# pastas/metran

Measured on AMD Instinct MI355X. Metric: Kalman filter+smoother steps/sec (batched DFMs), higher is better.
Workload: dtype f64

## Files before the change

### metran_amd/csrc/mk_kernels.hip

```cpp
#include <cstdlib>
#include <cstring>

#include "mk_prims.h"

namespace mk {

template <int n, int G, bool SYM>
struct RecordIO;
#ifndef MK_WIDE_FILTER_WAVES
#define MK_WIDE_FILTER_WAVES 2
#endif
#ifndef MK_WIDE_FILTER_LOOP
#define MK_WIDE_FILTER_LOOP 1
#endif
#ifndef MK_FILTER_LDS_STORES
#define MK_FILTER_LDS_STORES 1
#endif

template <int N, int K, int G, int OUT, bool BOOK, bool SYM>
__global__ void __launch_bounds__(256) __attribute__((amdgpu_waves_per_eu(G == 64 && N + K <= 40 ? MK_WIDE_FILTER_WAVES : 1))) filter_kernel(FilterArgs a)
{
    static_assert(!SYM || OUT == 1 || OUT == 3, "packed-symmetric layout applies to record outputs");
    constexpr int n = N + K;
    static_assert(n <= G, "state dimension must fit the lane group");
    constexpr bool TAPE = (OUT == 4);
    static_assert(!TAPE || (G == 64 && MK_WIDE_FILTER_LOOP && N * K > 32), "the tape leaves the one-model-per-wavefront loop filter");
    using Gp = Group<G>;
    constexpr int GPB = 256 / G;
    constexpr bool HOIST = (N * K <= 32);
    constexpr int NV = record_payload(n);
    const int lane = threadIdx.x % G;
    long inst = (long)blockIdx.x * GPB + threadIdx.x / G;
    if (inst > a.B - 1) inst = a.B - 1;
    const long rec = inst % a.R;
    const int r = lane < n ? lane : n - 1;
    const bool lead = lane == 0;
    const long T = a.T;

    const double phi_r = a.phi[inst * n + r];
    const double q_r = a.q[inst * n + r];
    constexpr bool WIDE = (G == 64);
    double pp[WIDE ? 1 : n], qd[WIDE ? 1 : n];
    constexpr int NP = n + (n & 1);
    __shared__ __attribute__((aligned(16))) double lds_phi[WIDE ? (256 / G) * 3 * NP : 1];
    double *phim = lds_phi + (WIDE ? (threadIdx.x / G) * 3 * NP : 0);
    double *dvec = phim + (WIDE ? NP : 0);
    double *dvec2 = dvec;
    if constexpr (WIDE) {
        phim[r] = phi_r;
        wave_lds_sync();
    } else {
        sfor<0, n>(MK_LAMBDA(c) {
            pp[decltype(c)::value] = phi_r * Gp::template bcast<decltype(c)::value>(phi_r);
            qd[decltype(c)::value] = (decltype(c)::value == r) ? q_r : 0.0;
        });
    }
    const int jr = lane < N ? lane : N - 1;
    double gam[K];
#pragma unroll
    for (int k = 0; k < K; ++k) gam[k] = a.loadings[(rec * N + jr) * K + k];
    const double rvar = a.obsvar ? a.obsvar[rec * N + jr] : 0.0;
    constexpr bool GTAB = WIDE && !HOIST;
    __shared__ __attribute__((aligned(16))) double lds_gam[GTAB ? (256 / G) * N * K : 1];
    double *gtab = lds_gam + (GTAB ? (threadIdx.x / G) * N * K : 0);
    if constexpr (GTAB) {
        if (lane < N) {
#pragma unroll
            for (int k = 0; k < K; ++k) gtab[lane * K + k] = gam[k];
        }
        wave_lds_sync();
    }
    double Gh[HOIST ? N : 1][K];
    if constexpr (HOIST) {
        sfor<0, N>(MK_LAMBDA(j) {
            sfor<0, K>(MK_LAMBDA(k) {
                Gh[decltype(j)::value][decltype(k)::value] = Gp::template bcast<decltype(j)::value>(gam[decltype(k)::value]);
            });
        });
    }

    double x = a.x0 ? a.x0[inst * n + r] : 0.0;
    double P[n];
#pragma unroll
    for (int c = 0; c < n; ++c) P[c] = a.P0 ? a.P0[(inst * n + r) * n + c] : (c == r ? 1.0 : 0.0);

    constexpr bool XREP = WIDE && MK_WIDE_FILTER_LOOP;
    double xk[XREP ? K : 1], phik[XREP ? K : 1];
    if constexpr (XREP) {
        sfor<0, K>(MK_LAMBDA(k) {
            xk[decltype(k)::value] = Gp::template bcast<N + decltype(k)::value>(x);
            phik[decltype(k)::value] = Gp::template bcast<N + decltype(k)::value>(phi_r);
        });
    }

    constexpr bool RECF = (OUT == 1 || OUT == 3);
    MomentPtr oP = moment_ptr<n>(a.Xp, a.Pp, inst * a.bs, a.ts, OUT == 1 ? a.rs : 0, r);
    MomentPtr oF = moment_ptr<n>(a.F, a.Pf, inst * a.bs, a.ts, RECF ? a.rs : 0, r);
    constexpr int RS = SYM ? record_stride_sym_c(n) : record_stride_c(n), NVO = SYM ? record_payload_sym(n) : NV;
    constexpr int PADN = RS - NVO;
    const int pslot = lane < PADN ? lane : PADN - 1;
    double *padF = RECF ? a.F + inst * a.bs * RS + NVO + pslot : nullptr;
    double *padP = OUT == 1 ? a.Xp + inst * a.bs * RS + NVO + pslot : nullptr;
    constexpr bool LDSOUT = MK_FILTER_LDS_STORES && RECF && G == 16;
    using RIO = RecordIO<n, G, SYM>;
    __shared__ __attribute__((aligned(16))) double lds_rec[LDSOUT ? 4 * 2 * RIO::LDS_PER_WAVE : 1];
    double *imgP = lds_rec + (LDSOUT ? (threadIdx.x / 64) * 2 * RIO::LDS_PER_WAVE : 0);
    double *imgF = imgP + (LDSOUT ? RIO::LDS_PER_WAVE : 0);
    const int lane64 = threadIdx.x & 63, gw = lane64 / G;
    typename RIO::Map rmap;
    double *recP = a.Xp, *recF = a.F;
    const long rstep = a.ts * RS;
    if constexpr (LDSOUT) {
        rmap = RIO::make_map(lane64, (long)blockIdx.x * GPB + (threadIdx.x / 64) * RIO::GW, a.B, a.bs);
        RIO::clear_tail(imgP, lane64);
        RIO::clear_tail(imgF, lane64);
        RIO::put_pad(imgP, gw, 0.0, 0.0);
    }
    double pad0 = 0.0, pad1 = 0.0;
    [[maybe_unused]] constexpr int XS = tape_xs_c(N, K);
    [[maybe_unused]] double *trec = TAPE ? a.F + inst * a.bs * a.rs : nullptr;
    [[maybe_unused]] const long tstep = a.ts * a.rs;

    constexpr int TS = 16;
    const int lrow = lane < TS ? lane : TS - 1;
    constexpr bool OV2 = (N % 2 == 0);
    constexpr int ONC = OV2 ? N / 2 : N;
    using ochunk_t = typename std::conditional<OV2, v2d, double>::type;
    __shared__ __attribute__((aligned(16))) double lds_obs[(256 / G) * TS * N];
    double *otile = lds_obs + (threadIdx.x / G) * TS * N;
    const double *obase = a.obs + rec * a.obs_bs * N;
    const long ostep = a.obs_ts * N;
    ochunk_t oreg[WIDE ? 1 : ONC];
    long otr = 0;
    auto obs_issue = [&](long t0) __attribute__((always_inline)) {
        long tr = t0 + lrow;
        if (tr > T - 1) tr = T - 1;
        if constexpr (WIDE) {
            otr = tr;
        } else {
            const ochunk_t *src = reinterpret_cast<const ochunk_t *>(obase + tr * ostep);
#pragma unroll
            for (int i = 0; i < ONC; ++i) oreg[i] = src[i];
        }
    };
    auto obs_park = [&]() __attribute__((always_inline)) {
        ochunk_t *dst = reinterpret_cast<ochunk_t *>(otile + lrow * N);
        wave_lds_sync();
        if constexpr (WIDE) {
            const ochunk_t *src = reinterpret_cast<const ochunk_t *>(obase + otr * ostep);
#pragma unroll
            for (int i = 0; i < ONC; ++i) dst[i] = src[i];
        } else {
#pragma unroll
            for (int i = 0; i < ONC; ++i) dst[i] = oreg[i];
        }
        wave_lds_sync();
    };
    obs_issue(0);
    double ynext = 0.0;

    double sum_sig = 0.0, sum_det = 0.0;
    double run_mant = 1.0;
    long run_exp = 0;
    long nobs = 0, sc = 0;
    double fmin_seen = 1.0;

    for (long t0 = 0; t0 < T; t0 += TS) {
    obs_park();
    obs_issue(t0 + TS);
    ynext = otile[jr];
    const long tend = t0 + TS < T ? t0 + TS : T;
    for (long t = t0; t < tend; ++t) {
        const double y = ynext;
        {
            const int s1 = (int)(t - t0) + 1;
            ynext = otile[(s1 < TS ? s1 : TS - 1) * N + jr];
        }
        const unsigned long long ball = __ballot(lane < N && isfinite(y));
        const auto vm = Gp::group_bits(ball);

        x = phi_r * x;
        if constexpr (XREP) {
#pragma unroll
            for (int k = 0; k < K; ++k) xk[k] = phik[k] * xk[k];
        }
        if constexpr (WIDE) {
            int rv = r;
            double qv = q_r;
            asm volatile("" : "+v"(rv), "+v"(qv));
            double phc[n];
            load_row<n>(phim, phc);
#pragma unroll
            for (int c = 0; c < n; ++c) P[c] = fma(P[c] * phi_r, phc[c], c == rv ? qv : 0.0);
        } else {
#pragma unroll
            for (int c = 0; c < n; ++c) P[c] = fma(P[c], pp[c], qd[c]);
        }
        if constexpr (LDSOUT && OUT == 1) {
            RIO::put(imgP, gw, r, x, P);
        } else if constexpr (OUT == 1) {
            *oP.vec = x;
            if constexpr (SYM) store_cols_sym<n>(oP.mat - r, P, r);
            else store_cols<n>(oP.mat, P);
            *padP = 0.0;
            oP.advance_nn(1);
            padP += a.ts * RS;
        } else if constexpr (OUT == 2) {
            if (oP.vec) *oP.vec = x;
            if (oP.mat) store_cols<n>(oP.mat, P);
            oP.advance(1);
        }

        double sigma = 0.0, fmant = 1.0;
        int fexp = 0;
        auto update = MK_LAMBDA(jc) {
            constexpr int j = decltype(jc)::value;
            double vl = y - x;
            sfor<0, K>(MK_LAMBDA(k) {
                constexpr int kk = decltype(k)::value;
                Gp::template fmac<N + kk, true>(vl, x, gam[kk]);
            });
            const double v = Gp::template bcast<j>(vl);
            double dr = P[j];
            sfor<0, K>(MK_LAMBDA(k) {
                constexpr int kk = decltype(k)::value;
                double g;
                if constexpr (HOIST) g = Gh[j][kk];
                else if constexpr (GTAB) g = gtab[j * K + kk];
                else g = Gp::template bcast<j>(gam[kk]);
                dr = fma(P[N + kk], g, dr);
            });
            double fl = rvar + dr;
            if constexpr (G == 16) dpp_pin(dr);
            sfor<0, K>(MK_LAMBDA(k) {
                constexpr int kk = decltype(k)::value;
                Gp::template fmac<N + kk, false>(fl, dr, gam[kk]);
            });
            const double f = Gp::template bcast<j>(fl);
            const double rf = rcp_nr(f);
            const double kr = dr * rf;
            if constexpr (WIDE) {
                dvec[r] = dr;
                wave_lds_sync();
                double dc[n];
                load_row<n>(dvec, dc);
#pragma unroll
                for (int c = 0; c < n; ++c) P[c] = fma(-dc[c], kr, P[c]);
            } else {
                Gp::template axpy_col<0, n, true, n>(P, dr, kr);
            }
            x = fma(kr, v, x);
            sigma = fma(v * v, rf, sigma);
            fmant *= f;
            if constexpr ((j & 3) == 3 || j == N - 1) {
                fexp += __builtin_amdgcn_frexp_exp(fmant);
                fmant = __builtin_amdgcn_frexp_mant(fmant);
            }
            fmin_seen = min_f64(fmin_seen, f);
        };
        if constexpr (WIDE && MK_WIDE_FILTER_LOOP) {
            unsigned long long m = (unsigned long long)vm;
            int nupd = 0;
            while (m) {
                const int j = __builtin_amdgcn_readfirstlane((int)__builtin_ctzll(m));
                m &= m - 1;
                double vl = y - x, vl2 = 0.0;
                sfor<0, K>(MK_LAMBDA(k) {
                    constexpr int kk = decltype(k)::value;
                    if constexpr (kk % 2 == 0) vl = fma(-gam[kk], xk[kk], vl);
                    else vl2 = fma(-gam[kk], xk[kk], vl2);
                });
                vl += vl2;
                const double v = readlane_f64(vl, j);
                double dr = 0.0;
                switch (j) {
#define MK_CASE_P(c) \
    case c:          \
        if constexpr (c < N) dr = P[c]; \
        break;
                    MK_CASE_P(0) MK_CASE_P(1) MK_CASE_P(2) MK_CASE_P(3) MK_CASE_P(4) MK_CASE_P(5) MK_CASE_P(6) MK_CASE_P(7)
                    MK_CASE_P(8) MK_CASE_P(9) MK_CASE_P(10) MK_CASE_P(11) MK_CASE_P(12) MK_CASE_P(13) MK_CASE_P(14) MK_CASE_P(15)
                    MK_CASE_P(16) MK_CASE_P(17) MK_CASE_P(18) MK_CASE_P(19) MK_CASE_P(20) MK_CASE_P(21) MK_CASE_P(22) MK_CASE_P(23)
                    MK_CASE_P(24) MK_CASE_P(25) MK_CASE_P(26) MK_CASE_P(27) MK_CASE_P(28) MK_CASE_P(29) MK_CASE_P(30) MK_CASE_P(31)
                    MK_CASE_P(32) MK_CASE_P(33) MK_CASE_P(34) MK_CASE_P(35) MK_CASE_P(36) MK_CASE_P(37) MK_CASE_P(38) MK_CASE_P(39)
                    MK_CASE_P(40) MK_CASE_P(41) MK_CASE_P(42) MK_CASE_P(43) MK_CASE_P(44) MK_CASE_P(45) MK_CASE_P(46) MK_CASE_P(47)
                    MK_CASE_P(48) MK_CASE_P(49) MK_CASE_P(50) MK_CASE_P(51) MK_CASE_P(52) MK_CASE_P(53) MK_CASE_P(54) MK_CASE_P(55)
                    MK_CASE_P(56) MK_CASE_P(57) MK_CASE_P(58) MK_CASE_P(59) MK_CASE_P(60) MK_CASE_P(61) MK_CASE_P(62) MK_CASE_P(63)
#undef MK_CASE_P
                default: break;
                }
                const double *gj = (GTAB ? gtab : dvec) + j * K;
                sfor<0, K>(MK_LAMBDA(k) {
                    constexpr int kk = decltype(k)::value;
                    double g;
                    if constexpr (GTAB) g = gj[kk];
                    else g = readlane_f64(gam[kk], j);
                    dr = fma(P[N + kk], g, dr);
                });
                double *dv = dvec2 + (nupd & 1) * NP;
                dv[r] = dr;
                double fl = rvar + dr, fl2 = 0.0;
                double dk[K];
                sfor<0, K>(MK_LAMBDA(k) { dk[decltype(k)::value] = Gp::template bcast<N + decltype(k)::value>(dr); });
                sfor<0, K>(MK_LAMBDA(k) {
                    constexpr int kk = decltype(k)::value;
                    if constexpr (kk % 2 == 0) fl = fma(dk[kk], gam[kk], fl);
                    else fl2 = fma(dk[kk], gam[kk], fl2);
                });
                fl += fl2;
                const double f = readlane_f64(fl, j);
                const double rf = rcp_nr(f);
                const double kr = dr * rf;
                if constexpr (OUT == 3 && !SYM) {
                    if (a.upd) {
                        double *ub = a.upd + (inst * a.bs + t * a.ts) * a.us + (long)nupd * adjoint_update_slot_c(N, K);
                        ub[r] = dr;
                        if (lead) *reinterpret_cast<v2d *>(ub + NP) = v2d{rf, v};
                    }
                }
                wave_lds_sync();
                {
                    double dc[n];
                    load_row<n>(dv, dc);
#pragma unroll
                    for (int c = 0; c < n; ++c) P[c] = fma(-dc[c], kr, P[c]);
                }
                if constexpr (TAPE) {
                    double kt = 0.0;
                    sfor<0, K>(MK_LAMBDA(k) { kt = fma(gam[decltype(k)::value], Gp::template bcast<N + decltype(k)::value>(kr), kt); });
                    kt = lane < N ? kr + kt : kr;
                    trec[j * XS + r] = kt;
                    const double yj = readlane_f64(y, j);
                    if (lead) {
                        double *sd = trec + j * XS + n;
                        sd[0] = v * rf;
                        sd[1] = rf;
                        sd[2] = yj;
                        sd[3] = 0.0;
                    }
                }
                sfor<0, K>(MK_LAMBDA(k) {
                    constexpr int kk = decltype(k)::value;
                    xk[kk] = fma(Gp::template bcast<N + kk>(kr), v, xk[kk]);
                });
                x = fma(kr, v, x);
                sigma = fma(v * v, rf, sigma);
                fmant *= f;
                if ((++nupd & 3) == 0) {
                    fexp += __builtin_amdgcn_frexp_exp(fmant);
                    fmant = __builtin_amdgcn_frexp_mant(fmant);
                }
                fmin_seen = min_f64(fmin_seen, f);
            }
            fexp += __builtin_amdgcn_frexp_exp(fmant);
            fmant = __builtin_amdgcn_frexp_mant(fmant);
        } else if (ball == Gp::full_mask(N)) {
            sfor<0, N>(update);
        } else {
            sfor<0, N>(MK_LAMBDA(jc) {
                if ((vm >> decltype(jc)::value) & 1) {
                    update(jc);
                } else if constexpr ((decltype(jc)::value & 3) == 3 || decltype(jc)::value == N - 1) {
                    fexp += __builtin_amdgcn_frexp_exp(fmant);
                    fmant = __builtin_amdgcn_frexp_mant(fmant);
                }
            });
        }

        const int cnt = __popcll((unsigned long long)vm);
        double pad = 0.0;
        if (cnt > 0) {
            if constexpr (BOOK) {
                int le;
                const double lm = log_mant(fmant, le);
                const double detf = fma((double)(fexp + le), kLn2, lm);
                if constexpr (RECF) {
                    if (sc == t) {
                        pad = pslot == 0 ? sigma : (pslot == 1 ? detf : 0.0);
                        pad0 = sigma;
                        pad1 = detf;
                    } else if (lead && a.sigmas)
                        *reinterpret_cast<v2d *>(a.F + (inst * a.bs + sc * a.ts) * RS + NVO) = v2d{sigma, detf};
                } else {
                    if (a.sigmas && lead) a.sigmas[(inst * a.bs + sc * a.ts) * a.sig_stride] = sigma;
                    if (a.detfs && lead) a.detfs[(inst * a.bs + sc * a.ts) * a.sig_stride] = detf;
                }
                if (sc >= a.warmup) {
                    sum_det += detf;
                    sum_sig += sigma;
                }
            } else {
                if (sc >= a.warmup) {
                    sum_sig += sigma;
                    run_mant *= fmant;
                    run_exp += fexp + __builtin_amdgcn_frexp_exp(run_mant);
                    run_mant = __builtin_amdgcn_frexp_mant(run_mant);
                }
            }
            ++sc;
        }
        if (t >= a.warmup) nobs += cnt;

        if constexpr (TAPE) {
            const double qnan = __builtin_nan("");
            if (a.tape == 2) {
                sfor<0, K>(MK_LAMBDA(kc) {
                    constexpr int k = decltype(kc)::value;
                    double qk = 0.0;
                    sfor<0, K>(MK_LAMBDA(k2) { qk = fma(gam[decltype(k2)::value], Gp::template bcast<N + decltype(k2)::value>(P[N + k]), qk); });
                    qk = lane < N ? P[N + k] + qk : P[N + k];
                    trec[(N + k) * XS + r] = qk;
                    const double pkk = Gp::template bcast<N + k>(P[N + k]);
                    if (lead) {
                        double *sd = trec + (N + k) * XS + n;
                        sd[0] = xk[k];
                        sd[1] = pkk;
                        sd[2] = qnan;
                        sd[3] = 0.0;
                    }
                });
            }
            unsigned long long um = ~(unsigned long long)vm & Gp::full_mask(N);
            double yh = x;
            sfor<0, K>(MK_LAMBDA(k) { yh = fma(gam[decltype(k)::value], xk[decltype(k)::value], yh); });
            while (um) {
                const int u = __builtin_amdgcn_readfirstlane((int)__builtin_ctzll(um));
                um &= um - 1;
                double dr = 0.0;
                switch (u) {
#define MK_CASE_PU(c) \
    case c:           \
        if constexpr (c < N) dr = P[c]; \
        break;
                    MK_CASE_PU(0) MK_CASE_PU(1) MK_CASE_PU(2) MK_CASE_PU(3) MK_CASE_PU(4) MK_CASE_PU(5) MK_CASE_PU(6) MK_CASE_PU(7) MK_CASE_PU(8) MK_CASE_PU(9) MK_CASE_PU(10) MK_CASE_PU(11) MK_CASE_PU(12) MK_CASE_PU(13) MK_CASE_PU(14) MK_CASE_PU(15) MK_CASE_PU(16) MK_CASE_PU(17) MK_CASE_PU(18) MK_CASE_PU(19) MK_CASE_PU(20) MK_CASE_PU(21) MK_CASE_PU(22) MK_CASE_PU(23) MK_CASE_PU(24) MK_CASE_PU(25) MK_CASE_PU(26) MK_CASE_PU(27) MK_CASE_PU(28) MK_CASE_PU(29) MK_CASE_PU(30) MK_CASE_PU(31) MK_CASE_PU(32) MK_CASE_PU(33) MK_CASE_PU(34) MK_CASE_PU(35) MK_CASE_PU(36) MK_CASE_PU(37) MK_CASE_PU(38) MK_CASE_PU(39) MK_CASE_PU(40) MK_CASE_PU(41) MK_CASE_PU(42) MK_CASE_PU(43) MK_CASE_PU(44) MK_CASE_PU(45) MK_CASE_PU(46) MK_CASE_PU(47) MK_CASE_PU(48) MK_CASE_PU(49) MK_CASE_PU(50) MK_CASE_PU(51) MK_CASE_PU(52) MK_CASE_PU(53) MK_CASE_PU(54) MK_CASE_PU(55) MK_CASE_PU(56) MK_CASE_PU(57) MK_CASE_PU(58) MK_CASE_PU(59) MK_CASE_PU(60) MK_CASE_PU(61) MK_CASE_PU(62) MK_CASE_PU(63)
#undef MK_CASE_PU
                default: break;
                }
                const double *gu = gtab + u * K;
                sfor<0, K>(MK_LAMBDA(k) { dr = fma(P[N + decltype(k)::value], gu[decltype(k)::value], dr); });
                double pt = 0.0;
                sfor<0, K>(MK_LAMBDA(k) { pt = fma(gam[decltype(k)::value], Gp::template bcast<N + decltype(k)::value>(dr), pt); });
                pt = lane < N ? dr + pt : dr;
                trec[u * XS + r] = pt;
                const double s0 = readlane_f64(yh, u), s1 = readlane_f64(pt, u);
                if (lead) {
                    double *sd = trec + u * XS + n;
                    sd[0] = s0;
                    sd[1] = s1;
                    sd[2] = qnan;
                    sd[3] = 0.0;
                }
            }
            trec += tstep;
        }

        if constexpr (LDSOUT) {
            RIO::put(imgF, gw, r, x, P);
            RIO::put_pad(imgF, gw, pad0, pad1);
            pad0 = pad1 = 0.0;
            if constexpr (OUT == 1) {
                RIO::emit2(imgP, recP, imgF, recF, rmap);
                recP += rstep;
            } else {
                RIO::emit(imgF, recF, rmap);
            }
            recF += rstep;
        } else if constexpr (RECF) {
            *oF.vec = x;
            if constexpr (SYM) store_cols_sym<n>(oF.mat - r, P, r);
            else store_cols<n>(oF.mat, P);
            *padF = pad;
            oF.advance_nn(1);
            padF += a.ts * RS;
        } else if constexpr (OUT == 2) {
            if (oF.vec) *oF.vec = x;
            if (oF.mat) store_cols<n>(oF.mat, P);
            oF.advance(1);
        }
    }
    }

    if (BOOK && !RECF) {
        for (long i = sc + lane; i < T; i += G) {
            if (a.sigmas) a.sigmas[(inst * a.bs + i * a.ts) * a.sig_stride] = 0.0;
            if (a.detfs) a.detfs[(inst * a.bs + i * a.ts) * a.sig_stride] = 0.0;
        }
    }
    if (lead) {
        if (!BOOK) sum_det = fma((double)run_exp, kLn2, log(run_mant));
        const bool bad_f = !(fmin_seen > 0.0) || x != x;
        if (a.mle) a.mle[inst] = bad_f ? __builtin_nan("") : ((double)nobs * kLog2Pi + sum_det) + sum_sig;
        if (a.sigmacount) a.sigmacount[inst] = sc;
        if (a.status) a.status[inst] = bad_f ? MK_FLAG_NONPOSITIVE_F : 0u;
    }
}

#ifndef MK_NT_IO
#define MK_NT_IO 1
#endif
template <class V>
__device__ __forceinline__ void rec_store(V *p, V v)
{
#if MK_NT_IO
    __builtin_nontemporal_store(v, p);
#else
    *p = v;
#endif
}
template <class V>
__device__ __forceinline__ V rec_load(const V *p)
{
#if MK_NT_IO
    return __builtin_nontemporal_load(p);
#else
    return *p;
#endif
}

template <int n, int G, bool SYM>
struct RecordIO {
    static constexpr int NV = n + n * n;
    static constexpr int RS = record_stride_c(n);
    static constexpr int NVO = SYM ? record_payload_sym(n) : NV;
    static constexpr int RSO = SYM ? record_stride_sym_c(n) : RS;
    static constexpr int RC = RSO / 2;
    static constexpr int GW = 64 / G;
    static constexpr int CW = GW * RC;
    static constexpr int PER = (CW + 63) / 64;
    static constexpr int SPARE = GW * RS;
    static constexpr int LDS_PER_WAVE = GW * RS + (SYM ? 2 : 0);
    using chunk_t = v2d;

    struct Map {
        long off[PER];
        int lq[PER];
        int a0[SYM ? PER : 1], a1[SYM ? PER : 1];
        int b0[SYM ? PER : 1], b1[SYM ? PER : 1];
        int m0[SYM ? PER : 1], m1[SYM ? PER : 1];
    };
    static __device__ __forceinline__ void locate(int p, int &pos, int &mirror, int &kind)
    {
        kind = 0;
        if (p < n) {
            pos = mirror = p;
        } else if (p < NVO) {
            int u = p - n, r = 0;
            while (u >= n - r) {
                u -= n - r;
                ++r;
            }
            const int c = r + u;
            pos = n + r * n + c;
            mirror = n + c * n + r;
        } else if (p < NVO + 2) {
            pos = mirror = NV + (p - NVO);
            kind = 1;
        } else {
            pos = mirror = 0;
            kind = 2;
        }
    }
    static __device__ __forceinline__ Map make_map(int lane64, long inst0, long B, long bs)
    {
        Map mp;
#pragma unroll
        for (int m = 0; m < PER; ++m) {
            int q = lane64 + 64 * m;
            if (q > CW - 1) q = CW - 1;
            const int g = q / RC, w = q - g * RC;
            long ig = inst0 + g;
            if (ig > B - 1) ig = B - 1;
            mp.off[m] = ig * bs * RSO + 2 * w;
            mp.lq[m] = q;
            if constexpr (SYM) {
                int pos, mir, kind;
                locate(2 * w, pos, mir, kind);
                mp.a0[m] = kind == 2 ? SPARE : g * RS + pos;
                mp.b0[m] = kind == 0 ? g * RS + pos : SPARE;
                mp.m0[m] = kind == 0 ? g * RS + mir : SPARE;
                locate(2 * w + 1, pos, mir, kind);
                mp.a1[m] = kind == 2 ? SPARE + 1 : g * RS + pos;
                mp.b1[m] = kind == 0 ? g * RS + pos : SPARE + 1;
                mp.m1[m] = kind == 0 ? g * RS + mir : SPARE + 1;
            }
        }
        return mp;
    }
    static __device__ __forceinline__ void put(double *img, int g, int r, double x, const double (&row)[n])
    {
        img[g * RS + r] = x;
        store_row<n>(img + g * RS + n + r * n, row);
    }
    static __device__ __forceinline__ void put_pad(double *img, int g, double s0, double s1)
    {
        *reinterpret_cast<v2d *>(img + g * RS + NV) = v2d{s0, s1};
    }
    static __device__ __forceinline__ void clear_tail(double *img, int lane64)
    {
        for (int i = lane64; i < GW * (RS - NV - 2); i += 64) {
            const int g = i / (RS - NV - 2 > 0 ? RS - NV - 2 : 1), w = i % (RS - NV - 2 > 0 ? RS - NV - 2 : 1);
            img[g * RS + NV + 2 + w] = 0.0;
        }
        if constexpr (SYM)
            if (lane64 < 2) img[SPARE + lane64] = 0.0;
    }
    static __device__ __forceinline__ chunk_t gather(const double *img, const Map &mp, int m)
    {
        if constexpr (SYM) return chunk_t{img[mp.a0[m]], img[mp.a1[m]]};
        else return reinterpret_cast<const chunk_t *>(img)[mp.lq[m]];
    }
    static __device__ __forceinline__ void emit(const double *img, double *base, const Map &mp)
    {
        chunk_t tmp[PER];
        gather_all(img, mp, tmp);
        store_all(base, mp, tmp);
    }
    static __device__ __forceinline__ void gather_all(const double *img, const Map &mp, chunk_t (&tmp)[PER])
    {
        wave_lds_sync();
#pragma unroll
        for (int m = 0; m < PER; ++m) tmp[m] = gather(img, mp, m);
    }
    static __device__ __forceinline__ void store_all(double *base, const Map &mp, const chunk_t (&tmp)[PER])
    {
#pragma unroll
        for (int m = 0; m < PER; ++m) rec_store(reinterpret_cast<chunk_t *>(base + mp.off[m]), tmp[m]);
    }
    static __device__ __forceinline__ void emit2(const double *img0, double *base0, const double *img1, double *base1,
                                                 const Map &mp)
    {
        wave_lds_sync();
        chunk_t t0[PER], t1[PER];
#pragma unroll
        for (int m = 0; m < PER; ++m) {
            t0[m] = gather(img0, mp, m);
            t1[m] = gather(img1, mp, m);
        }
#pragma unroll
        for (int m = 0; m < PER; ++m) rec_store(reinterpret_cast<chunk_t *>(base0 + mp.off[m]), t0[m]);
#pragma unroll
        for (int m = 0; m < PER; ++m) rec_store(reinterpret_cast<chunk_t *>(base1 + mp.off[m]), t1[m]);
    }
    static __device__ __forceinline__ void load_issue(const double *base, const Map &mp, chunk_t (&buf)[PER])
    {
#pragma unroll
        for (int m = 0; m < PER; ++m) buf[m] = rec_load(reinterpret_cast<const chunk_t *>(base + mp.off[m]));
    }
    static __device__ __forceinline__ void to_image(double *img, const chunk_t (&buf)[PER], const Map &mp)
    {
        wave_lds_sync();
        if constexpr (SYM) {
#pragma unroll
            for (int m = 0; m < PER; ++m) {
                img[mp.b0[m]] = buf[m].x;
                img[mp.b1[m]] = buf[m].y;
                img[mp.m0[m]] = buf[m].x;
                img[mp.m1[m]] = buf[m].y;
            }
        } else {
            chunk_t *l = reinterpret_cast<chunk_t *>(img);
#pragma unroll
            for (int m = 0; m < PER; ++m) l[mp.lq[m]] = buf[m];
        }
        wave_lds_sync();
    }
    static __device__ __forceinline__ void load_finish(double *img, const chunk_t (&buf)[PER], const Map &mp, int g,
                                                       int r, double &x, double (&row)[n])
    {
        to_image(img, buf, mp);
        x = img[g * RS + r];
        load_row<n>(img + g * RS + n + r * n, row);
    }
};

template <int N, int K, int G, int EPI, bool SYM>
__global__ void __launch_bounds__(256) smoother_record_kernel(SmootherArgs a)
{
    constexpr bool PROJ = (EPI == 1), VAR = (EPI == 2);
    constexpr int n = N + K;
    static_assert(n <= G, "state dimension must fit the lane group");
    using Gp = Group<G>;
    constexpr int GPB = 256 / G;
    const int lane = threadIdx.x % G;
    long inst = (long)blockIdx.x * GPB + threadIdx.x / G;
    const bool live = inst < a.B;
    if (!live) inst = a.B - 1;
    const int r = lane < n ? lane : n - 1;
    const long T = a.T;

    const double phi_r = a.phi[inst * n + r];
    const double q_r = a.q[inst * n + r];
    double phic[n], qd[n];
    sfor<0, n>(MK_LAMBDA(c) {
        phic[decltype(c)::value] = Gp::template bcast<decltype(c)::value>(phi_r);
        qd[decltype(c)::value] = (decltype(c)::value == r) ? q_r : 0.0;
    });

    constexpr bool REC = true;
    using RIO = RecordIO<n, G, SYM>;
    constexpr int LDS_DOUBLES = 4 * 2 * RIO::LDS_PER_WAVE;
    __shared__ __attribute__((aligned(16))) double lds_io[LDS_DOUBLES];
    const int lane64 = threadIdx.x & 63;
    const int gw = lane64 / G;
    double *imgL = lds_io + (threadIdx.x / 64) * 2 * RIO::LDS_PER_WAVE;
    double *imgS = imgL + RIO::LDS_PER_WAVE;
    typename RIO::Map rmap;
    if constexpr (REC) {
        rmap = RIO::make_map(lane64, (long)blockIdx.x * GPB + (threadIdx.x / 64) * RIO::GW, a.B, a.bs);
        RIO::clear_tail(imgS, lane64);
        RIO::put_pad(imgS, gw, 0.0, 0.0);
    }
    typename RIO::chunk_t prer[RIO::PER];

    const long rstep = a.ts * RIO::RSO;
    const double *recF = a.F + (T - 1) * rstep;
    double *recS = a.S ? a.S + (T - 1) * rstep : nullptr;

    const long rec_id = inst % a.R;
    const int jr = lane < N ? lane : N - 1;
    double gam[K], pscale = 1.0, poffset = 0.0;
    double *pM = nullptr, *pV = nullptr;
    if constexpr (PROJ) {
#pragma unroll
        for (int k = 0; k < K; ++k) gam[k] = a.loadings[(rec_id * N + jr) * K + k];
        if (a.scale) pscale = a.scale[rec_id * N + jr];
        if (a.offset) poffset = a.offset[rec_id * N + jr];
        const long pidx = (inst * a.bs + (T - 1) * a.ts) * N + jr;
        pM = a.sim_means ? a.sim_means + pidx : nullptr;
        pV = a.sim_vars ? a.sim_vars + pidx : nullptr;
    }
    double *sM = nullptr, *sV = nullptr;
    if constexpr (VAR) {
        const long sidx = (inst * a.bs + (T - 1) * a.ts) * n + r;
        sM = a.state_means + sidx;
        sV = a.state_vars + sidx;
    }

    auto issue = [&](double &xnext) __attribute__((always_inline)) {
        recF -= rstep;
        RIO::load_issue(recF, rmap, prer);
    };
    auto finish = [&](double &xv, double(&row)[n]) __attribute__((always_inline)) {
        RIO::load_finish(imgL, prer, rmap, gw, r, xv, row);
    };
    constexpr bool DEFER = (EPI == 0);
    auto store = [&](double xv, const double(&row)[n]) __attribute__((always_inline)) {
        if (recS) {
            RIO::put(imgS, gw, r, xv, row);
            if constexpr (!DEFER) {
                RIO::emit(imgS, recS, rmap);
                recS -= rstep;
            }
        }
        if constexpr (PROJ) {
            double mean, var;
            project<N, K, G>(xv, row, gam, pscale, poffset, lane, mean, var);
            if (lane < N && live) {
                if (pM) *pM = mean;
                if (pV) *pV = var;
            }
            if (pM) pM -= a.ts * N;
            if (pV) pV -= a.ts * N;
        }
        if constexpr (VAR) {
            double diag = 0.0;
            sfor<0, n>(MK_LAMBDA(c) { diag = (decltype(c)::value == lane) ? row[decltype(c)::value] : diag; });
            if (lane < n && live) {
                *sM = xv;
                *sV = diag;
            }
            sM -= a.ts * n;
            sV -= a.ts * n;
        }
    };
    typename RIO::chunk_t etmp[RIO::PER];

    double xs, Psn[n];
    RIO::load_issue(recF, rmap, prer);
    finish(xs, Psn);
    store(xs, Psn);
    double pivmin = 1.0;

    double Pfc[n], xfc = 0.0, xfn = 0.0;
    if (T >= 2) {
        issue(xfc);
        finish(xfc, Pfc);
        if (T >= 3) issue(xfn);
    }

    for (long t = T - 2; t >= 0; --t) {
        double A[n], z[n], D[n];
#pragma unroll
        for (int c = 0; c < n; ++c) {
            z[c] = Pfc[c] * phic[c];
            A[c] = fma(phi_r, z[c], qd[c]);
            D[c] = Psn[c] - A[c];
            if constexpr (DEFER) Psn[c] = Pfc[c];
        }
        double delta = xs - phi_r * xfc;
        if constexpr (G == 16) dpp_pin(delta);

        if constexpr (DEFER)
            if (recS) RIO::gather_all(imgS, rmap, etmp);

        if constexpr (G == 16) dpp_guard(A);
        double dinv[n];
        ldlt_factor<n, G, false>(A, dinv, pivmin);
        if (__builtin_expect(__ballot(!(pivmin > 0.0)) != 0ull, 0)) {
#pragma unroll
            for (int c = 0; c < n; ++c) A[c] = fma(phi_r, z[c], qd[c]);
            if constexpr (G == 16) dpp_guard(A);
            ldlt_factor<n, G, true>(A, dinv, pivmin);
        }
        double xf_next = xfn;
        if constexpr (DEFER) {
            if (t >= 1) {
                finish(xf_next, Pfc);
                if (t >= 2) issue(xfn);
            }
            if (recS) {
                RIO::store_all(recS, rmap, etmp);
                recS -= rstep;
            }
        }

        constexpr bool FUSED = (G == 16) && Sweeps<n>::fused;
        if constexpr (FUSED) {
            Sweeps<n>::forward(z, A);
        } else {
            sfor<0, n>(MK_LAMBDA(kc) {
                constexpr int k = decltype(kc)::value;
                Gp::template axpy_col<k + 1, n, true, n>(z, A[k], z[k]);
            });
        }
#pragma unroll
        for (int c = 0; c < n; ++c) z[c] *= dinv[c];
        if constexpr (FUSED) {
            Sweeps<n>::backward(z, A);
        } else {
            sfor_down<0, n>(MK_LAMBDA(kc) {
                constexpr int k = decltype(kc)::value;
                Gp::template axpy_lane<k, 0, k, true, n>(z, A, z[k]);
            });
        }

        double acc0 = xfc, acc1 = 0.0;
        if constexpr (FUSED) {
            Sweeps<n>::mean(acc0, acc1, delta, z);
        } else {
            sfor<0, n>(MK_LAMBDA(cc) {
                constexpr int c = decltype(cc)::value;
                if constexpr (c % 2 == 0) Gp::template fmac<c>(acc0, delta, z[c]);
                else Gp::template fmac<c>(acc1, delta, z[c]);
            });
        }
        xs = acc0 + acc1;

        double V[n];
        if constexpr (G == 16) dpp_guard(D);
        if constexpr (FUSED) {
            Sweeps<n>::jd(V, D, z);
        } else {
#pragma unroll
            for (int c = 0; c < n; ++c) V[c] = 0.0;
            sfor<0, n>(MK_LAMBDA(kc) {
                constexpr int k = decltype(kc)::value;
                Gp::template axpy_lane<k, 0, n, false, n>(V, D, z[k]);
            });
        }
        if constexpr (!DEFER) {
#pragma unroll
            for (int c = 0; c < n; ++c) Psn[c] = Pfc[c];
        }
        if constexpr (FUSED) {
            Sweeps<n>::vjt(Psn, z, V);
        } else {
            sfor<0, n>(MK_LAMBDA(kc) {
                constexpr int k = decltype(kc)::value;
                Gp::template axpy_col<0, n, false, n>(Psn, z[k], V[k]);
            });
        }

        if constexpr (!DEFER) {
            if (t >= 1) {
                finish(xf_next, Pfc);
                if (t >= 2) issue(xfn);
            }
        }
        store(xs, Psn);
        xfc = xf_next;
    }
    if constexpr (DEFER)
        if (recS) RIO::emit(imgS, recS, rmap);
    if (a.status && live && lane == 0 && pivot_flags(pivmin)) atomicOr(a.status + inst, pivot_flags(pivmin));
}


template <int N, int K, bool SYM>
struct BlkLayout {
    static constexpr int n = N + K;
    using RIO = RecordIO<n, 16, SYM>;
    static constexpr int NBR = (n + 3) / 4;
    static constexpr int NBC = (n + 4) / 4;
    static constexpr int TR = 4 * NBR;
    static constexpr int TS = 20;
    static constexpr int IM = ((TR * TS - 8 + 31) / 32) * 32 + 8;
    static constexpr int DUMP = 4 * IM, ZERO = 4 * IM + 2;
    static constexpr int IMG = 4 * IM + 4;
    static constexpr int JR = 4 * NBR;
    static constexpr int JM = (n + 1) * JR;
    static constexpr int WAVE = 2 * IMG + 4 * JM;
    static_assert(n <= 15 && 4 * NBC <= TS, "the mean rides as column n of the tile");
    static_assert(IM % 2 == 0 && IMG % 2 == 0 && JM % 2 == 0 && JR % 2 == 0, "16-byte alignment of the row accesses");

    struct Map {
        long off[RIO::PER];
        int l0[RIO::PER], l1[RIO::PER];
        int s0[RIO::PER], s1[RIO::PER];
        int m0[SYM ? RIO::PER : 1], m1[SYM ? RIO::PER : 1];
    };
    static __device__ __forceinline__ void locate(int p, int &pos, int &mirror, int &kind)
    {
        if constexpr (SYM) {
            int rp, rm;
            RIO::locate(p, rp, rm, kind);
            pos = rp < n ? rp * TS + n : ((rp - n) / n) * TS + (rp - n) % n;
            mirror = rm < n ? rm * TS + n : ((rm - n) / n) * TS + (rm - n) % n;
        } else {
            kind = p < RIO::NV ? 0 : (p < RIO::NV + 2 ? 1 : 2);
// ... 1169 lines not shown
```

### metran_amd/jit.py

```python
import hashlib
import logging
import os
import shutil
import subprocess
import sys
import tempfile
import time

from . import _lib
from ._lib import MetranHipError

logger = logging.getLogger(__name__)
_HERE = os.path.dirname(os.path.abspath(__file__))
_ROOT = os.path.dirname(_HERE)
_SOURCES = [os.path.join(_HERE, "csrc", f) for f in ("mk_kernels.hip", "mk_wide.hip", "mk_split.hip", "mk_dk.hip",
                                                     "mk_internal.h", "mk_jump.h", "mk_prims.h", "mk_sweeps.h")] + [
    os.path.join(_ROOT, "include", "metran_hip.h")]


class ShapeUnavailable(MetranHipError):
    """No specialised module can be HAD for a shape -- no compiler on the machine, or ``METRAN_HIP_JIT=0`` -- which is not an
    error of anything: the caller may fall back to the size-generic kernels (``BatchedKalman._ensure_kernels``)."""


class ShapeBuildError(MetranHipError):
    """A module was attempted and FAILED -- hipcc, the linker, or the static hazard checks on its assembly.  Never a reason
    to fall back silently: a kernel regression or a hazard would go unnoticed behind kernels ten times slower."""


def _hipcc():
    for c in (os.environ.get("HIPCC"), shutil.which("hipcc"), "/opt/rocm/bin/hipcc"):
        if c and os.path.exists(c):
            return c
    raise ShapeUnavailable("hipcc not found: cannot build a kernel module for this model shape")


def cache_dir():
    d = os.environ.get("METRAN_HIP_CACHE") or os.path.join(os.path.expanduser("~"), ".cache", "metran_amd")
    os.makedirs(d, exist_ok=True)
    return d


def _extra_flags():
    return os.environ.get("METRAN_HIP_JIT_FLAGS", "").split()


def _source_hash():
    h = hashlib.sha256()
    for f in _SOURCES:
        data = open(f, "rb").read()
        if f.endswith("metran_hip.h"):
            data = b"\n".join(ln for ln in data.splitlines() if ln.startswith((b"#define MK_API", b"#define MK_FLAG_", b"#define MK_OUT_")))
        h.update(data)
    h.update(" ".join(_extra_flags()).encode())
    return h.hexdigest()[:16]


PREBUILT_DIR = os.path.join(_HERE, "_shape_cache")


def _module_name(N, K):
    return "mk_shape_%d_%d_%s.so" % (N, K, _source_hash())


def module_path(N, K):
    return os.path.join(cache_dir(), _module_name(N, K))


def prebuilt_path(N, K):
    return os.path.join(PREBUILT_DIR, _module_name(N, K))


def build_shape_module(N, K, out=None):
    if out is None:
        pre = prebuilt_path(N, K)
        if os.path.exists(pre):
            return pre
        out = module_path(N, K)
    if os.path.exists(out):
        return out
    if os.environ.get("METRAN_HIP_JIT", "1") == "0":
        raise ShapeUnavailable("no kernel for (N=%d, K=%d) and METRAN_HIP_JIT=0 forbids building one" % (N, K))
    n = N + K
    if N < 1 or K < 1 or n > 64:
        raise MetranHipError("unsupported model shape N=%d, K=%d (need N, K >= 1 and N + K <= 64)" % (N, K))
    logger.info("building HIP kernels for a %d-series / %d-factor model (one-off, cached)", N, K)
    t_start = time.perf_counter()
    tmp = tempfile.mkdtemp(prefix="mkjit_")
    try:
        hipcc = _hipcc()
        base = [hipcc, "--offload-arch=gfx950", "-O3", "-std=c++17", "-fPIC", "-fvisibility=hidden",
                "-I" + os.path.join(_ROOT, "include"), "-I" + os.path.join(_HERE, "csrc"), "-DMK_SHAPE_MODULE",
                "-DMK_SHAPES(X)=X(%d,%d)" % (N, K), "-save-temps=obj", "-Wno-unused-command-line-argument"] + _extra_flags()
        src = {os.path.basename(f): f for f in _SOURCES}
        units = [("kernels", src["mk_kernels.hip"], []), ("split", src["mk_split.hip"], []), ("dk", src["mk_dk.hip"], [])]
        units += ([("wide_p%d" % p_, src["mk_wide.hip"], ["-DMK_WIDE_PART=%d" % p_]) for p_ in range(7)] if n > 16
                  else [("wide", src["mk_wide.hip"], [])])

        def compile_unit(unit):
            name, source, flags = unit
            d = os.path.join(tmp, name)
            os.makedirs(d)
            obj = os.path.join(d, "unit.o")
            r = subprocess.run(base + flags + ["-c", source, "-o", obj], cwd=d, capture_output=True, text=True)
            if r.returncode != 0:
                raise ShapeBuildError("hipcc failed for shape (%d,%d), unit %s:\n%s" % (N, K, name, r.stderr[-2000:]))
            for f in os.listdir(d):
                if not f.endswith("gfx950.s"):
                    continue
                for script, what in (("check_dpp_hazards.py", "DPP"), ("check_asm_hazards.py", "inline-asm")):
                    checker = os.path.join(_ROOT, "scripts", script)
                    if os.path.exists(checker):
                        c = subprocess.run([sys.executable, checker, os.path.join(d, f)], capture_output=True, text=True)
                        if c.returncode != 0:
                            raise ShapeBuildError("%s hazard check failed for shape (%d,%d), unit %s:\n%s" % (what, N, K, name, c.stdout[-2000:]))
            return obj

        from concurrent.futures import ThreadPoolExecutor

        jobs = max(1, min(len(units), _UNIT_JOBS or int(os.environ.get("METRAN_HIP_JIT_JOBS", "0")) or (os.cpu_count() or 2)))
        with ThreadPoolExecutor(max_workers=jobs) as ex:
            objs = list(ex.map(compile_unit, units))
        so = os.path.join(tmp, "mod.so")
        r = subprocess.run([hipcc, "--offload-arch=gfx950", "-shared", "-fPIC", "-o", so] + objs, capture_output=True, text=True)
        if r.returncode != 0:
            raise ShapeBuildError("link failed for shape (%d,%d):\n%s" % (N, K, r.stderr[-2000:]))
        logger.info("kernels for (N=%d, K=%d) built in %.0f s (%d translation units, %d at a time)", N, K, time.perf_counter() - t_start,
                    len(units), jobs)
        fd, stage = tempfile.mkstemp(prefix=".mk_shape_", suffix=".so", dir=os.path.dirname(out))
        os.close(fd)
        shutil.copyfile(so, stage)
        os.chmod(stage, 0o755)
        os.replace(stage, out)
    finally:
        shutil.rmtree(tmp, ignore_errors=True)
    return out


def ensure_shape(N, K):
    L = _lib.lib()
    if L.mk_shape_specialised(N, K):
        return False
    path = build_shape_module(int(N), int(K))
    _lib.check(L.mk_register_shape_module(path.encode()))
    if not L.mk_shape_specialised(N, K):
        raise MetranHipError("shape module %s did not register (N=%d, K=%d)" % (path, N, K))
    return True


def parse_shapes(specs):
    out = []
    for spec in specs:
        a, b = spec.lower().split("x")
        rng = lambda t: range(int(t.split("-")[0]), int(t.split("-")[-1]) + 1)
        out += [(N, K) for N in rng(a) for K in rng(b)]
    return out


_UNIT_JOBS = 0


def prebuild(shapes, jobs=None, verbose=True, budget_s=None):
    global _UNIT_JOBS
    from concurrent.futures import ThreadPoolExecutor

    os.makedirs(PREBUILT_DIR, exist_ok=True)
    L = _lib.lib()
    todo = [(N, K) for (N, K) in dict.fromkeys(shapes) if not _aot(L, N, K) and N + K <= 64 and not os.path.exists(prebuilt_path(N, K))]
    cpus = os.cpu_count() or 2
    t0 = time.perf_counter()
    skipped, failed = [], []

    def one(shape):
        if budget_s is not None and time.perf_counter() - t0 > budget_s:
            skipped.append(shape)
            return None
        try:
            path = build_shape_module(shape[0], shape[1], out=prebuilt_path(*shape))
        except ShapeBuildError as e:
            failed.append((shape, str(e)))
            return None
        if verbose:
            print("%s  (%d,%d)  [%.0f s]" % (os.path.relpath(path, _ROOT), shape[0], shape[1], time.perf_counter() - t0), flush=True)
        return path

    out = []
    for group, at_once in (([sh for sh in todo if sh[0] + sh[1] > 16], jobs or 2), ([sh for sh in todo if sh[0] + sh[1] <= 16], jobs or max(1, cpus // 2))):
        if not group:
            continue
        at_once = max(1, min(at_once, len(group)))
        _UNIT_JOBS = max(1, cpus // at_once)
        try:
            with ThreadPoolExecutor(max_workers=at_once) as ex:
                out += [p_ for p_ in ex.map(one, group) if p_]
        finally:
            _UNIT_JOBS = 0
    if skipped and verbose:
        print("prebuild: time budget of %.0f s spent; not built (they compile at first use, or at the next prebuild): %s"
              % (budget_s, " ".join("%dx%d" % sh for sh in skipped)), flush=True)
    if failed:
        raise ShapeBuildError("%d shape module(s) failed to build:\n%s" % (len(failed), "\n".join("(%d,%d): %s" % (sh[0], sh[1], msg) for sh, msg in failed)))
    return out


GRID_SHAPES = [(N, K) for K in (1, 2, 3) for N in range(2, 17)] + [(20, 2), (24, 3), (32, 2), (32, 3), (32, 4)]


def _aot(L, N, K):
    import ctypes

    shapes = (ctypes.c_int64 * 512)()
    cnt = L.mk_supported_shapes(shapes, 256)
    aot = {(int(shapes[2 * i]), int(shapes[2 * i + 1])) for i in range(min(cnt, 256))}
    return (N, K) in aot


def prune():
    gone = []
    if os.path.isdir(PREBUILT_DIR):
        tag = "_%s.so" % _source_hash()
        for f in os.listdir(PREBUILT_DIR):
            if f.startswith("mk_shape_") and f.endswith(".so") and not f.endswith(tag):
                os.remove(os.path.join(PREBUILT_DIR, f))
                gone.append(f)
    return gone


TEST_SHAPES = [(7, 2), (11, 3), (14, 2), (20, 2), (16, 2), (32, 1), (48, 3), (17, 1), (17, 3), (20, 4), (11, 6), (12, 3), (9, 2), (19, 2),
               (12, 4), (13, 4), (20, 6), (23, 5), (33, 4), (40, 4), (59, 4), (60, 4)]


if __name__ == "__main__":
    import argparse

    ap = argparse.ArgumentParser(description="prebuild run-time shape modules into metran_amd/_shape_cache")
    ap.add_argument("shapes", nargs="*", help="e.g. 2-12x1-3 20x2")
    ap.add_argument("--tests", action="store_true", help="the shapes the GPU test tier uses")
    ap.add_argument("--grid", action="store_true", help="N = 2..16 x K = 1..3 plus (20,2) (24,3) (32,2..4): what build() prebuilds")
    ap.add_argument("--budget", type=float, default=None, help="seconds after which no new module is started")
    ap.add_argument("--jobs", type=int, default=None)
    ap.add_argument("--prune", action="store_true", help="remove modules built from other sources")
    a = ap.parse_args()
    if a.prune:
        for f in prune():
            print("removed", f)
    want = parse_shapes(a.shapes) + (TEST_SHAPES if a.tests else []) + (GRID_SHAPES if a.grid else [])
    if want:
        prebuild(want, jobs=a.jobs, budget_s=a.budget)
```

Measured before the change: 1.321 billion.

## Defer filter record stores and interleave them with the next step's updates

For small-state G=16 record-output filters, the LDS-staged record of step t is no longer gathered and stored at the end of the step. Its gather and global-store chunks are spread across the per-observation update slots of step t+1, so memory traffic overlaps the serial update chain. The log-determinant bookkeeping is also carried one step late to drop the log from the critical path, and waves_per_eu is raised to 2 for these shapes. This adds register pressure for the carried chunks, sched barriers that constrain the scheduler, and MK_TUNE_SKIP probe paths in the non-deferred branch.

```diff
diff --git a/metran_amd/csrc/mk_kernels.hip b/metran_amd/csrc/mk_kernels.hip
--- a/metran_amd/csrc/mk_kernels.hip
+++ b/metran_amd/csrc/mk_kernels.hip
@@ -16,9 +16,20 @@
 #ifndef MK_FILTER_LDS_STORES
 #define MK_FILTER_LDS_STORES 1
 #endif
+#ifndef MK_FILTER_DEFER
+#define MK_FILTER_DEFER 1
+#endif
+#ifndef MK_FILTER_DEFER_LOG
+#define MK_FILTER_DEFER_LOG 1
+#endif
+#define MK_FILTER_WAVES(n, NK, G, OUT) ((MK_FILTER_DEFER && MK_FILTER_LDS_STORES && (G) == 16 && ((OUT) == 1 || (OUT) == 3) && (n) <= 10 && (NK) <= 16) ? 2 : 1)
+template <int N>
+constexpr int filter_gather_slot(int q) { return q < N - 1 ? q : N - 1; }
+template <int N>
+constexpr int filter_store_slot(int q) { return filter_gather_slot<N>(q) + 1; }
 
 template <int N, int K, int G, int OUT, bool BOOK, bool SYM>
-__global__ void __launch_bounds__(256) __attribute__((amdgpu_waves_per_eu(G == 64 && N + K <= 40 ? MK_WIDE_FILTER_WAVES : 1))) filter_kernel(FilterArgs a)
+__global__ void __launch_bounds__(256) __attribute__((amdgpu_waves_per_eu(G == 64 && N + K <= 40 ? MK_WIDE_FILTER_WAVES : MK_FILTER_WAVES(N + K, N * K, G, OUT)))) filter_kernel(FilterArgs a)
 {
     static_assert(!SYM || OUT == 1 || OUT == 3, "packed-symmetric layout applies to record outputs");
     constexpr int n = N + K;
@@ -115,8 +126,69 @@
         RIO::clear_tail(imgP, lane64);
         RIO::clear_tail(imgF, lane64);
         RIO::put_pad(imgP, gw, 0.0, 0.0);
+        if constexpr (MK_FILTER_DEFER) {
+            RIO::put(imgF, gw, r, x, P);
+            RIO::put_pad(imgF, gw, 0.0, 0.0);
+        }
     }
     double pad0 = 0.0, pad1 = 0.0;
+    double sum_sig = 0.0, sum_det = 0.0;
+    long sc = 0;
+    constexpr bool FDEFER = MK_FILTER_DEFER && LDSOUT;
+    constexpr bool FDLOG = FDEFER && BOOK && MK_FILTER_DEFER_LOG && !(SYM && OUT == 1);
+    constexpr int FPER = RIO::PER;
+    constexpr int FNC = (OUT == 1 ? 2 : 1) * FPER;
+    double c_sigma = 0.0, c_fmant = 1.0;
+    int c_fexp = 0;
+    bool c_has = false;
+    typename RIO::chunk_t ch[FNC];
+    double *recFc = a.F;
+    auto carried_book = [&](long tc) __attribute__((always_inline)) {
+        if (c_has) {
+            const long csc = sc - 1;
+            int le;
+            const double lm = log_mant(c_fmant, le);
+            const double detf = fma((double)(c_fexp + le), kLn2, lm);
+            if (csc == tc) {
+                pad0 = c_sigma;
+                pad1 = detf;
+            } else if (lead && a.sigmas) {
+                *reinterpret_cast<v2d *>(a.F + (inst * a.bs + csc * a.ts) * RS + NVO) = v2d{c_sigma, detf};
+            }
+            if (csc >= a.warmup) {
+                sum_det += detf;
+                sum_sig += c_sigma;
+            }
+        }
+        RIO::put_pad(imgF, gw, pad0, pad1);
+        pad0 = pad1 = 0.0;
+    };
+    auto chunk_store = [&](auto qc) __attribute__((always_inline)) {
+        constexpr int q = decltype(qc)::value, m = OUT == 1 ? q / 2 : q;
+        __builtin_amdgcn_sched_barrier(0);
+        if constexpr (OUT == 1 && q % 2 == 0) {
+            RIO::store_one(recP, rmap, m, ch[q]);
+        } else {
+            RIO::store_one(recFc, rmap, m, ch[q]);
+        }
+    };
+    auto slot = MK_LAMBDA(jc) {
+        if constexpr (FDEFER) {
+            constexpr int j = decltype(jc)::value;
+            sfor<0, FNC>(MK_LAMBDA(qc) {
+                if constexpr (filter_store_slot<N>(decltype(qc)::value) == j) chunk_store(qc);
+            });
+            sfor<0, FNC>(MK_LAMBDA(qc) {
+                constexpr int q = decltype(qc)::value, m = OUT == 1 ? q / 2 : q;
+                if constexpr (filter_gather_slot<N>(q) == j) {
+                    __builtin_amdgcn_sched_barrier(0);
+                    wave_lds_sync();
+                    ch[q] = RIO::gather((OUT == 1 && q % 2 == 0) ? imgP : imgF, rmap, m);
+                }
+            });
+            __builtin_amdgcn_sched_barrier(0);
+        }
+    };
     [[maybe_unused]] constexpr int XS = tape_xs_c(N, K);
     [[maybe_unused]] double *trec = TAPE ? a.F + inst * a.bs * a.rs : nullptr;
     [[maybe_unused]] const long tstep = a.ts * a.rs;
@@ -159,10 +231,9 @@
     obs_issue(0);
     double ynext = 0.0;
 
-    double sum_sig = 0.0, sum_det = 0.0;
     double run_mant = 1.0;
     long run_exp = 0;
-    long nobs = 0, sc = 0;
+    long nobs = 0;
     double fmin_seen = 1.0;
 
     for (long t0 = 0; t0 < T; t0 += TS) {
@@ -211,6 +282,7 @@
             oP.advance(1);
         }
 
+        if constexpr (FDLOG) carried_book(t - 1);
         double sigma = 0.0, fmant = 1.0;
         int fexp = 0;
         auto update = MK_LAMBDA(jc) {
@@ -355,7 +427,10 @@
             fexp += __builtin_amdgcn_frexp_exp(fmant);
             fmant = __builtin_amdgcn_frexp_mant(fmant);
         } else if (ball == Gp::full_mask(N)) {
-            sfor<0, N>(update);
+            sfor<0, N>(MK_LAMBDA(jc) {
+                update(jc);
+                slot(jc);
+            });
         } else {
             sfor<0, N>(MK_LAMBDA(jc) {
                 if ((vm >> decltype(jc)::value) & 1) {
@@ -364,16 +439,24 @@
                     fexp += __builtin_amdgcn_frexp_exp(fmant);
                     fmant = __builtin_amdgcn_frexp_mant(fmant);
                 }
+                slot(jc);
             });
         }
 
         const int cnt = __popcll((unsigned long long)vm);
         double pad = 0.0;
-        if (cnt > 0) {
+        if constexpr (FDEFER && !FDLOG) slot(std::integral_constant<int, N>{});
+        if constexpr (FDLOG) {
+            c_has = cnt > 0;
+            c_sigma = sigma;
+            c_fmant = fmant;
+            c_fexp = fexp;
+            if (cnt > 0) ++sc;
+        } else if (cnt > 0) {
             if constexpr (BOOK) {
-                int le;
-                const double lm = log_mant(fmant, le);
-                const double detf = fma((double)(fexp + le), kLn2, lm);
+                int le = 0;
+                const double lm = MK_TUNE_SKIP(a, 4) ? 0.5 : log_mant(fmant, le);
+                const double detf = MK_TUNE_SKIP(a, 4) ? lm : fma((double)(fexp + le), kLn2, lm);
                 if constexpr (RECF) {
                     if (sc == t) {
                         pad = pslot == 0 ? sigma : (pslot == 1 ? detf : 0.0);
@@ -454,11 +537,48 @@
             trec += tstep;
         }
 
-        if constexpr (LDSOUT) {
+        if constexpr (FDEFER) {
+            RIO::put(imgF, gw, r, x, P);
+            if constexpr (!FDLOG) {
+                RIO::put_pad(imgF, gw, pad0, pad1);
+                pad0 = pad1 = 0.0;
+            }
+            if constexpr (FDLOG) slot(std::integral_constant<int, N>{});
+            if constexpr (OUT == 1) recP += rstep;
+            recFc = recF;
+            recF += rstep;
+        } else if constexpr (LDSOUT) {
             RIO::put(imgF, gw, r, x, P);
             RIO::put_pad(imgF, gw, pad0, pad1);
             pad0 = pad1 = 0.0;
-            if constexpr (OUT == 1) {
+            if constexpr (MK_TUNE_SKIP(a, 1) || MK_TUNE_SKIP(a, 2)) {
+                typename RIO::chunk_t tP[FPER], tF[FPER];
+                if constexpr (MK_TUNE_SKIP(a, 2)) {
+#pragma unroll
+                    for (int m = 0; m < FPER; ++m) tP[m] = tF[m] = typename RIO::chunk_t{P[(2 * m) % n], P[(2 * m + 1) % n]};
+                } else {
+                    wave_lds_sync();
+#pragma unroll
+                    for (int m = 0; m < FPER; ++m) {
+                        if constexpr (OUT == 1) tP[m] = RIO::gather(imgP, rmap, m);
+                        tF[m] = RIO::gather(imgF, rmap, m);
+                    }
+                }
+#pragma unroll
+                for (int m = 0; m < FPER; ++m) {
+                    if constexpr (MK_TUNE_SKIP(a, 1)) {
+                        if constexpr (OUT == 1) asm volatile("" ::"v"(tP[m]));
+                        asm volatile("" ::"v"(tF[m]));
+                    } else {
+                        if constexpr (OUT == 1) RIO::store_one(recP, rmap, m, tP[m]);
+                    }
+                }
+                if constexpr (!MK_TUNE_SKIP(a, 1)) {
+#pragma unroll
+                    for (int m = 0; m < FPER; ++m) RIO::store_one(recF, rmap, m, tF[m]);
+                }
+                if constexpr (OUT == 1) recP += rstep;
+            } else if constexpr (OUT == 1) {
                 RIO::emit2(imgP, recP, imgF, recF, rmap);
                 recP += rstep;
             } else {
@@ -480,6 +600,12 @@
     }
     }
 
+    if constexpr (FDEFER) {
+        if (T > 0) {
+            if constexpr (FDLOG) carried_book(T - 1);
+            RIO::emit(imgF, recFc, rmap);
+        }
+    }
     if (BOOK && !RECF) {
         for (long i = sc + lane; i < T; i += G) {
             if (a.sigmas) a.sigmas[(inst * a.bs + i * a.ts) * a.sig_stride] = 0.0;
@@ -625,6 +751,10 @@
     {
 #pragma unroll
         for (int m = 0; m < PER; ++m) rec_store(reinterpret_cast<chunk_t *>(base + mp.off[m]), tmp[m]);
+    }
+    static __device__ __forceinline__ void store_one(double *base, const Map &mp, int m, chunk_t v)
+    {
+        rec_store(reinterpret_cast<chunk_t *>(base + mp.off[m]), v);
     }
     static __device__ __forceinline__ void emit2(const double *img0, double *base0, const double *img1, double *base1,
                                                  const Map &mp)
diff --git a/metran_amd/jit.py b/metran_amd/jit.py
--- a/metran_amd/jit.py
+++ b/metran_amd/jit.py
@@ -227,7 +227,8 @@
 
 
 TEST_SHAPES = [(7, 2), (11, 3), (14, 2), (20, 2), (16, 2), (32, 1), (48, 3), (17, 1), (17, 3), (20, 4), (11, 6), (12, 3), (9, 2), (19, 2),
-               (12, 4), (13, 4), (20, 6), (23, 5), (33, 4), (40, 4), (59, 4), (60, 4)]
+               (12, 4), (13, 4), (20, 6), (23, 5), (33, 4), (40, 4), (59, 4), (60, 4),
+               (1, 1)]
 
 
 if __name__ == "__main__":
```

New measurement: 1.345 billion (median of 6 runs). 1.02x the previous value.
